# sgl-project/rbg

Hardware: AMD Instinct MI355X
Metric: output tok/s (llama-3-8b P/D-disagg serving, KV migration over xGMI) (higher is better)
Workload: dtype bf16; 1 GPU; model=llama-3-8b, global_batch=128, seq_len=2048, parallelism=pd1 (1 prefill + 1 decode, prefill colocated with decode0)

## Files before the change

rbg_amd/models/llama.py:

```python
from __future__ import annotations

import math
from dataclasses import dataclass
from typing import Optional

import torch
import torch.nn as nn

from .. import ops
from ..engine.config import ModelConfig
from ..engine.kv_cache import PagedKVCache


@dataclass
class ForwardBatch:
    mode: str
    positions: torch.Tensor
    slot_mapping: torch.Tensor
    cu_seqlens: Optional[torch.Tensor] = None
    cu_seqlens_k: Optional[torch.Tensor] = None
    kv_gather_slots: Optional[torch.Tensor] = None
    block_tables: Optional[torch.Tensor] = None
    context_lens: Optional[torch.Tensor] = None
    decode_num_splits: int = 0
# ... 105 lines not shown
                                 requires_grad=False)
        self.wo = _linear_weight(cfg.hidden_size, full_q, device, dtype, gen,
                                 shard_dim=1, tp_size=tp.size,
                                 tp_rank=tp.rank)
        self.q_out, self.kv_out = q_out, kv_out
        self.q_norm = self.k_norm = None
        if cfg.qk_norm:
            self.q_norm = nn.Parameter(torch.ones(cfg.head_dim, device=device,
                                                  dtype=dtype),
                                       requires_grad=False)
            self.k_norm = nn.Parameter(torch.ones(cfg.head_dim, device=device,
                                                  dtype=dtype),
                                       requires_grad=False)

    def forward(self, x: torch.Tensor, batch: ForwardBatch,
                kv: PagedKVCache, cos_sin: torch.Tensor,
                add_norm=None) -> torch.Tensor:
        T = x.shape[0]
        qkv = ops.linear(x, self.wqkv)
        q = qkv[:, :self.q_out]
        k = qkv[:, self.q_out:self.q_out + self.kv_out]
        v = qkv[:, self.q_out + self.kv_out:]
        if self.q_norm is not None:
            q = ops.rmsnorm(q.contiguous().view(-1, self.head_dim),
                            self.q_norm,
                            self.cfg.rms_eps).view(T, self.q_out)
            k = ops.rmsnorm(k.contiguous().view(-1, self.head_dim),
                            self.k_norm,
                            self.cfg.rms_eps).view(T, self.kv_out)
            v = v.clone(memory_format=torch.contiguous_format)
        key_cache = kv.key_cache(self.layer_idx)
        value_cache = kv.value_cache(self.layer_idx)
        fp8 = kv.fp8
        if fp8:
            ops.rope_store_kv(q, k, v, key_cache, value_cache, cos_sin,
                              batch.positions, batch.slot_mapping,
                              kv.k_scale_log2, kv.v_scale_log2)
        else:
            ops.rope_store_kv(q, k, v, key_cache, value_cache, cos_sin,
                              batch.positions, batch.slot_mapping)
        q3 = q.view(T, self.heads, self.head_dim)
        if batch.mode == "prefill":
            if fp8:
                if batch.kv_gather_slots is None:
                    raise RuntimeError("an fp8 KV pool prefills through the "
                                       "gather path: kv_gather_slots unset")
                k_full = ops.kv_gather_dequant(
                    key_cache, batch.kv_gather_slots, kv.k_scale_log2)
                v_full = ops.kv_gather_dequant(
                    value_cache, batch.kv_gather_slots, kv.v_scale_log2)
                o = ops.prefill_attention(q3, k_full, v_full,
                                          batch.cu_seqlens, self.scale,
                                          batch.cu_seqlens_k)
            elif batch.kv_gather_slots is not None:
                ps = key_cache.shape[2]
                slots = batch.kv_gather_slots.long()
                pages, offs = slots // ps, slots % ps
                k_full = key_cache[pages, :, offs]
                v_full = value_cache[pages, :, offs]
                o = ops.prefill_attention(q3, k_full, v_full,
                                          batch.cu_seqlens, self.scale,
                                          batch.cu_seqlens_k)
            else:
                o = ops.prefill_attention(
                    q3, k.view(T, self.kv_heads, self.head_dim),
                    v.view(T, self.kv_heads, self.head_dim),
                    batch.cu_seqlens, self.scale)
        elif fp8:
            o = ops.decode_attention(q3, key_cache, value_cache,
                                     batch.block_tables, batch.context_lens,
                                     self.scale,
                                     num_splits=batch.decode_num_splits,
                                     k_scale_log2=kv.k_scale_log2,
                                     v_scale_log2=kv.v_scale_log2)
        else:
            o = ops.decode_attention(q3, key_cache, value_cache,
                                     batch.block_tables, batch.context_lens,
                                     self.scale,
                                     num_splits=batch.decode_num_splits)
        o = o.view(T, self.q_out).contiguous()
        if add_norm is not None:
            return ops.linear_add_rmsnorm(o, self.wo, *add_norm)
        return self.tp.all_reduce(ops.linear(o, self.wo))


class LlamaMLP(nn.Module):
    def __init__(self, cfg: ModelConfig, tp: TPContext, device, dtype, gen):
        super().__init__()
        self.tp = tp
        assert cfg.intermediate_size % tp.size == 0
        inter = cfg.intermediate_size // tp.size
        wg = _linear_weight(cfg.intermediate_size, cfg.hidden_size, device,
                            dtype, gen, shard_dim=0, tp_size=tp.size,
                            tp_rank=tp.rank)
        wu = _linear_weight(cfg.intermediate_size, cfg.hidden_size, device,
                            dtype, gen, shard_dim=0, tp_size=tp.size,
                            tp_rank=tp.rank)
        self.w_gate_up = nn.Parameter(torch.cat([wg, wu], dim=0),
                                      requires_grad=False)
        self.w_down = _linear_weight(cfg.hidden_size, cfg.intermediate_size,
                                     device, dtype, gen, shard_dim=1,
                                     tp_size=tp.size, tp_rank=tp.rank)
        self.inter = inter

    def forward(self, x: torch.Tensor, add_norm=None) -> torch.Tensor:
        gu = ops.linear(x, self.w_gate_up)
        h = ops.silu_mul(gu)
        if add_norm is not None:
            return ops.linear_add_rmsnorm(h, self.w_down, *add_norm)
        return self.tp.all_reduce(ops.linear(h, self.w_down))


# ... 135 lines not shown
```

rbg_amd/ops/__init__.py:

```python
from __future__ import annotations

import os

import torch

from . import reference

_hip = None
_hip_err: Exception | None = None
try:
    from . import _hip_ops as _hip
except Exception as e:
    _hip_err = e

HAVE_HIP = _hip is not None


def _check_stale() -> None:
    import hashlib
    here = os.path.dirname(os.path.abspath(__file__))
    stamp = os.path.join(here, "_hip_ops.srchash")
    if not os.path.exists(stamp):
        return
    h = hashlib.sha256()
# ... 117 lines not shown


def kv_gather_dequant(cache, slots, scale_log2: int = 0) -> torch.Tensor:
    if cache.dtype != FP8:
        raise ValueError("kv_gather_dequant needs a float8_e4m3fn cache, "
                         "got %s" % cache.dtype)
    check_kv_scale_log2(scale_log2, "scale_log2")
    if _on_gpu(cache):
        return _require_hip().kv_gather_dequant(cache, slots, scale_log2)
    return reference.kv_gather_dequant(cache, slots, scale_log2)


def pick_decode_splits(num_seqs: int, num_kv_heads: int,
                       max_context: int, variant: int = -1) -> int:
    if variant < 0:
        variant = DECODE_VARIANT
    if variant >= 4:
        per_wg = 2 if variant in (4, 5) else 1
        base = num_kv_heads * ((num_seqs + per_wg - 1) // per_wg)
        by_ctx = max(1, max_context // 32)
    else:
        base = num_seqs * num_kv_heads
        by_ctx = max(1, max_context // 256)
    if base >= 1024:
        return 1
    want = max(1, 1024 // max(base, 1))
    return int(min(want, by_ctx, 16))


DECODE_VARIANT = int(os.environ.get("RBG_DECODE_VARIANT", "4"))
PREFILL_SWZ = int(os.environ.get("RBG_PREFILL_SWZ", "6"))


def decode_attention(q, key_cache, value_cache, block_tables, context_lens,
                     scale: float, num_splits: int = 0,
                     variant: int = -1, k_scale_log2: int = 0,
                     v_scale_log2: int = 0) -> torch.Tensor:
    if _is_fp8_pair(key_cache, value_cache):
        if variant not in (-1, 4):
            raise ValueError("an fp8 KV cache has no decode variant %d: only "
                             "variant 4 reads e4m3" % variant)
        check_kv_scale_log2(k_scale_log2, "kv_k_scale_log2")
        check_kv_scale_log2(v_scale_log2, "kv_v_scale_log2")
        if key_cache.shape[2] != 16 or key_cache.shape[3] != 128:
            raise ValueError("fp8 decode needs page size 16 and head_dim 128, "
                             "got %d and %d" % (key_cache.shape[2],
                                                key_cache.shape[3]))
        if _on_gpu(q):
            if num_splits <= 0:
                max_ctx = (int(context_lens.max().item())
                           if context_lens.numel() else 1)
                num_splits = pick_decode_splits(q.shape[0],
                                                key_cache.shape[1], max_ctx, 4)
            return _require_hip().decode_attention_fp8(
                q, key_cache, value_cache, block_tables, context_lens, scale,
                num_splits, k_scale_log2, v_scale_log2)
        return reference.decode_attention(
            q, key_cache, value_cache, block_tables, context_lens, scale,
            k_scale_log2, v_scale_log2)
    if _on_gpu(q):
        if num_splits <= 0:
            max_ctx = int(context_lens.max().item()) if context_lens.numel() else 1
            num_splits = pick_decode_splits(q.shape[0], key_cache.shape[1],
                                            max_ctx)
        if variant < 0:
            variant = DECODE_VARIANT
        return _require_hip().decode_attention(
            q, key_cache, value_cache, block_tables, context_lens, scale,
            num_splits, variant)
    return reference.decode_attention(q, key_cache, value_cache, block_tables,
                                      context_lens, scale)


def prefill_attention(q, k, v, cu_seqlens, scale: float,
                      cu_seqlens_k=None) -> torch.Tensor:
    if _on_gpu(q):
        qtile = 128 if (PREFILL_SWZ & 12) else 64
        block_info, seq_lens = reference.prefill_block_info(
            cu_seqlens.cpu(), qtile=qtile,
            cu_seqlens_k=None if cu_seqlens_k is None else cu_seqlens_k.cpu())
        return _require_hip().prefill_attention(
            q, k, v, block_info.to(q.device), seq_lens.to(q.device), scale,
            PREFILL_SWZ)
    return reference.prefill_attention(q, k, v, cu_seqlens, scale,
                                       cu_seqlens_k)


build_cos_sin_table = reference.build_cos_sin_table


def sample(logits, temperature, top_k, top_p, min_p, seed, pos):
    if _on_gpu(logits):
        toks, kept = _require_hip().sample(logits, temperature, top_k, top_p,
                                           min_p, seed, pos)
        return toks, kept
    return reference.sample(logits, temperature, top_k, top_p, min_p, seed,
                            pos)
```

rbg_amd/ops/hip/attn_decode.hip:

```cpp
#include "attn_mfma.h"

namespace {

struct SplitRange { int key_begin, key_end, pg_begin, pg_end; };

DEV_INLINE SplitRange split_range(int ctx, int split, int num_splits) {
  const int chunk = 16;
  const int nchunks = (ctx + chunk - 1) / chunk;
  const int per_split = (nchunks + num_splits - 1) / num_splits;
  SplitRange r;
  r.key_begin = split * per_split * chunk;
  r.key_end = min(ctx, (split + 1) * per_split * chunk);
  r.pg_begin = r.key_begin >> 4;
  r.pg_end = (r.key_end + 15) >> 4;
  return r;
}

template <int QPG, int VARIANT>
__global__ __launch_bounds__(256,
    (VARIANT == 3) ? 4 : ((VARIANT >= 1 && QPG <= 4) ? 5 : 2))
void decode_attn_kernel(
    float* __restrict__ partial_o,
    float* __restrict__ partial_ml,
    __hip_bfloat16* __restrict__ out,
    const __hip_bfloat16* __restrict__ q,
    const __hip_bfloat16* __restrict__ key_cache,
    const __hip_bfloat16* __restrict__ val_cache,
    const int* __restrict__ block_tables,
    const int* __restrict__ context_lens,
    const float scale, const int num_kv_heads, const int page_size,
    const int max_pages, const int num_splits, const int q_stride) {
  const int kvh = blockIdx.x;
  const int seq = blockIdx.y;
  const int split = blockIdx.z;
  const int num_q_heads = num_kv_heads * QPG;
// ... 303 lines not shown
    }
  }
}

#define DM_REGS(R) uint4 R##0, R##1, R##2, R##3, R##4, R##5, R##6, R##7
#define DM_ISSUE(cache, R, pg)                                              \
  do {                                                                      \
    const int p_ = btab[min((pg) + myloc, pg_last)];                        \
    const __hip_bfloat16* src_ = (cache) + schunk +                         \
        (((size_t)p_ * num_kv_heads + kvh) * 16 + (srow & 15)) * HEAD_DIM;  \
    R##0 = *reinterpret_cast<const uint4*>(src_);                           \
    R##1 = *reinterpret_cast<const uint4*>(src_ + 8);                       \
    R##2 = *reinterpret_cast<const uint4*>(src_ + 16);                      \
    R##3 = *reinterpret_cast<const uint4*>(src_ + 24);                      \
    R##4 = *reinterpret_cast<const uint4*>(src_ + 32);                      \
    R##5 = *reinterpret_cast<const uint4*>(src_ + 40);                      \
    R##6 = *reinterpret_cast<const uint4*>(src_ + 48);                      \
    R##7 = *reinterpret_cast<const uint4*>(src_ + 56);                      \
  } while (0)
#define DM_K_AT(c) (&k_lds[srow * DM_KP + schunk + (c)])
#define DM_V_AT(c) (&v_img[v_img_off(srow, schunk + (c))])
#define DM_WRITE(R, AT)                                                     \
  do {                                                                      \
    *reinterpret_cast<uint4*>(AT(0)) = R##0;                                \
    *reinterpret_cast<uint4*>(AT(8)) = R##1;                                \
    *reinterpret_cast<uint4*>(AT(16)) = R##2;                               \
    *reinterpret_cast<uint4*>(AT(24)) = R##3;                               \
    *reinterpret_cast<uint4*>(AT(32)) = R##4;                               \
    *reinterpret_cast<uint4*>(AT(40)) = R##5;                               \
    *reinterpret_cast<uint4*>(AT(48)) = R##6;                               \
    *reinterpret_cast<uint4*>(AT(56)) = R##7;                               \
  } while (0)

template <int QPG, int DIET>
__global__ __launch_bounds__(128, DIET ? 4 : 3) void decode_attn_mfma_kernel(
    float* __restrict__ partial_o,
    float* __restrict__ partial_ml,
    __hip_bfloat16* __restrict__ out,
    const __hip_bfloat16* __restrict__ q,
    const __hip_bfloat16* __restrict__ key_cache,
    const __hip_bfloat16* __restrict__ val_cache,
    const int* __restrict__ block_tables,
    const int* __restrict__ context_lens,
    const float scale, const int num_kv_heads, const int max_pages,
    const int num_splits, const int num_seqs, const int q_stride) {
  const int kvh = blockIdx.x;
  const int wave = threadIdx.x >> 6;
  const int seq = blockIdx.y * 2 + wave;
  const int split = blockIdx.z;
  const int lane = threadIdx.x & 63;
  const int gl = lane & 15;
  const int gslice = lane >> 4;

  __shared__ __hip_bfloat16 kv_all[2][32 * DM_KP];
  __shared__ __hip_bfloat16 p_lds_all[2][16 * DM_PP];
  __hip_bfloat16* k_lds = kv_all[wave];
  __hip_bfloat16* v_img = kv_all[wave];
  __hip_bfloat16* p_lds = p_lds_all[wave];
  if (seq >= num_seqs) return;
  const SplitRange sr = split_range(context_lens[seq], split, num_splits);

  const __hip_bfloat16* q_seq = q + (size_t)seq * q_stride;
  bf8 qa[4];
  if constexpr (!DIET) load_q_frags<QPG>(qa, q_seq, kvh, gl, gslice);

  const int* btab = block_tables + (size_t)seq * max_pages;
  const int srow = lane >> 1, schunk = (lane & 1) * 64, myloc = srow >> 4;
  const int pg_last = max(sr.pg_end - 1, 0);
  DM_REGS(ka);

  float m[4], l[4];
  f32x4 acc_o[8];
#pragma unroll
  for (int r = 0; r < 4; ++r) { m[r] = NEG_INF; l[r] = 0.f; }
#pragma unroll
  for (int dt = 0; dt < 8; ++dt) acc_o[dt] = {0.f, 0.f, 0.f, 0.f};

  DM_ISSUE(key_cache, ka, sr.pg_begin);

  for (int pg = sr.pg_begin; pg < sr.pg_end; pg += 2) {
    if constexpr (DIET) load_q_frags<QPG>(qa, q_seq, kvh, gl, gslice);
    DM_WRITE(ka, DM_K_AT);
    DM_REGS(va);
    if constexpr (!DIET) DM_ISSUE(val_cache, va, pg);
    asm volatile("s_waitcnt lgkmcnt(0)" ::: "memory");

    f32x4 sA, sB;
    score_pair(sA, sB, qa, k_lds, gl, gslice);
    if constexpr (DIET) DM_ISSUE(val_cache, va, pg);

    pair_softmax(sA, sB, scale, pg, sr, m, l, acc_o, p_lds, gl, gslice);
    DM_WRITE(va, DM_V_AT);
    DM_ISSUE(key_cache, ka, pg + 2);
    asm volatile("s_waitcnt lgkmcnt(0)" ::: "memory");

    const bf8 pa = load_p_frag(p_lds, gl, gslice);
    const unsigned vaddr = v_img_lane_addr(v_img, gl, gslice);
    if constexpr (!DIET) {
      PV_STEP16(acc_o, pa, vaddr);
    } else {
      PV_STEP8(acc_o, pa, vaddr, 0);
      PV_STEP8(acc_o, pa, vaddr, 1);
    }
  }

  store_pair_output<QPG>(partial_o, partial_ml, out, acc_o, m, l, seq,
                         num_seqs, split, num_splits, kvh, num_kv_heads, gl,
                         gslice);
}

template <int QPG>
__global__ __launch_bounds__(128, 4) void decode_attn_pc_kernel(
    float* __restrict__ partial_o,
    float* __restrict__ partial_ml,
    __hip_bfloat16* __restrict__ out,
    const __hip_bfloat16* __restrict__ q,
    const __hip_bfloat16* __restrict__ key_cache,
    const __hip_bfloat16* __restrict__ val_cache,
    const int* __restrict__ block_tables,
    const int* __restrict__ context_lens,
    const float scale, const int num_kv_heads, const int max_pages,
    const int num_splits, const int num_seqs, const int q_stride) {
  const int kvh = blockIdx.x;
  const int seq = blockIdx.y;
  const int split = blockIdx.z;
  const int wave = threadIdx.x >> 6;
  const int lane = threadIdx.x & 63;
  const int gl = lane & 15;
  const int gslice = lane >> 4;

  __shared__ __hip_bfloat16 k_lds[32 * DM_KP];
  __shared__ __hip_bfloat16 v_img[32 * 128];
  __shared__ __hip_bfloat16 p_lds[16 * DM_PP];
  __shared__ int flags[4];
  if (threadIdx.x == 0) {
    flags[0] = -1; flags[1] = -1; flags[2] = -1; flags[3] = -1;
  }
  __syncthreads();
  volatile int* f_prod_k = &flags[0];
  volatile int* f_prod_v = &flags[1];
  volatile int* f_cons_s = &flags[2];
// ... 180 lines not shown
#pragma unroll
    for (int r = 0; r < 4; ++r) acc_o[dt][r] *= v_scale;

  store_pair_output<QPG>(partial_o, partial_ml, out, acc_o, m, l, seq,
                         num_seqs, split, num_splits, kvh, num_kv_heads, gl,
                         gslice);
}

#undef DQ_REGS
#undef DQ_ISSUE
#undef DQ_WRITE1
#undef DQ_WRITE
#undef DM_REGS
#undef DM_ISSUE
#undef DM_K_AT
#undef DM_V_AT
#undef DM_WRITE

__global__ void decode_combine_kernel(
    __hip_bfloat16* __restrict__ out,
    const float* __restrict__ partial_o,
    const float* __restrict__ partial_ml,
    const int num_splits, const int num_q_heads) {
  const int seq = blockIdx.x, qh = blockIdx.y, d = threadIdx.x;
  const int seqs = gridDim.x;
  float m_star = NEG_INF;
  for (int s = 0; s < num_splits; ++s)
    m_star = fmaxf(m_star,
                   partial_ml[(((size_t)s * seqs + seq) * num_q_heads + qh) * 2]);
  float o = 0.f, lsum = 0.f;
  for (int s = 0; s < num_splits; ++s) {
    const float* ml =
        partial_ml + (((size_t)s * seqs + seq) * num_q_heads + qh) * 2;
    const float f = __expf(ml[0] - m_star);
    o += partial_o[(((size_t)s * seqs + seq) * num_q_heads + qh) * HEAD_DIM +
                   d] * f;
    lsum += ml[1] * f;
  }
  out[((size_t)seq * num_q_heads + qh) * HEAD_DIM + d] =
      f2bf(lsum > 0.f ? o / lsum : 0.f);
}

typedef void (*DecodeKernel)(float*, float*, __hip_bfloat16*,
                             const __hip_bfloat16*, const __hip_bfloat16*,
                             const __hip_bfloat16*, const int*, const int*,
                             float, int, int, int, int, int);

template <int QPG>
DecodeKernel decode_kernel(int variant) {
  switch (variant) {
    case 0: return decode_attn_kernel<QPG, 0>;
    case 1: return decode_attn_kernel<QPG, 1>;
    case 2: return decode_attn_kernel<QPG, 2>;
    case 3: return decode_attn_kernel<QPG, 3>;
    case 4: return decode_attn_mfma_kernel<QPG, 0>;
    case 5: return decode_attn_mfma_kernel<QPG, 1>;
    case 6: return decode_attn_pc_kernel<QPG>;
    default: return nullptr;
  }
}

}

extern "C" {

void launch_decode_attention(void* out, void* partial_o, void* partial_ml,
                             const void* q, const void* key_cache,
                             const void* val_cache, const void* block_tables,
                             const void* context_lens, float scale,
                             int num_seqs, int num_q_heads, int num_kv_heads,
                             int page_size, int max_pages, int num_splits,
                             int variant, int q_stride, hipStream_t stream) {
  const int qpg = num_q_heads / num_kv_heads;
  const bool mfma = variant >= 4 && variant <= 6 && page_size == 16;
  const int v = (mfma || (variant >= 0 && variant <= 3)) ? variant : 1;
  const DecodeKernel kernel = qpg == 1   ? decode_kernel<1>(v)
                              : qpg == 2 ? decode_kernel<2>(v)
                              : qpg == 4 ? decode_kernel<4>(v)
                              : qpg == 8 ? decode_kernel<8>(v)
                                         : nullptr;
  if (kernel == nullptr) return;
  const int seq_blocks = (v == 4 || v == 5) ? (num_seqs + 1) / 2 : num_seqs;
  const dim3 grid(num_kv_heads, seq_blocks, num_splits);
  const dim3 block(mfma ? 128 : 256);
  hipLaunchKernelGGL(kernel, grid, block, 0, stream, (float*)partial_o,
                     (float*)partial_ml, (__hip_bfloat16*)out,
                     (const __hip_bfloat16*)q,
                     (const __hip_bfloat16*)key_cache,
                     (const __hip_bfloat16*)val_cache,
                     (const int*)block_tables, (const int*)context_lens,
                     scale, num_kv_heads, mfma ? max_pages : page_size,
                     mfma ? num_splits : max_pages,
                     mfma ? num_seqs : num_splits, q_stride);
  if (num_splits > 1) {
    dim3 cgrid(num_seqs, num_q_heads), cblock(HEAD_DIM);
    hipLaunchKernelGGL(decode_combine_kernel, cgrid, cblock, 0, stream,
                       (__hip_bfloat16*)out, (const float*)partial_o,
// ... 41 lines not shown
```

rbg_amd/ops/hip/bindings.cpp:

```cpp
#include <torch/extension.h>
#include <ATen/hip/HIPContext.h>

#include <hip/hip_runtime.h>

#include <algorithm>
#include <cmath>
#include <cstring>
#include <vector>

extern "C" {
void launch_rmsnorm(void*, void*, const void*, float, int, int, hipStream_t);
void launch_fused_add_rmsnorm(void*, void*, const void*, float, int, int,
                              hipStream_t);
void launch_silu_mul(void*, const void*, int, int, hipStream_t);
void launch_rope_store_kv(void*, void*, const void*, void*, void*,
                          const void*, const void*, const void*, int, int,
                          int, int, int, int, int, hipStream_t);
void launch_decode_attention(void*, void*, void*, const void*, const void*,
                             const void*, const void*, const void*, float,
                             int, int, int, int, int, int, int, int,
                             hipStream_t);
void launch_prefill_attention(void*, const void*, const void*, const void*,
                              const void*, const void*, float, int, int, int,
                              int, int, int, hipStream_t);
void launch_mfma_probe(void*, const void*, const void*, int, int, hipStream_t);
void launch_mfma_probe32(void*, const void*, const void*, int, int, int,
                         hipStream_t);
void launch_skinny_gemm(void*, void*, const void*, const void*, int, int,
                        int, int, hipStream_t);
void launch_skinny_gemm_wide(void*, void*, const void*, const void*, int, int,
                             int, int, hipStream_t);
void launch_reduce_splits(void*, const void*, int, long, hipStream_t);
void launch_fold_add_rmsnorm(void*, const void*, void*, const void*, float,
                             int, int, int, hipStream_t);
void launch_kv_peer_copy(void*, const void*, const void*, const void*, int,
                         int, int, long, long, long, long, hipStream_t);
void launch_xgmi_allreduce(void*, const void*, void**, void**, int, int,
                           long, hipStream_t);
void launch_sample(void*, void*, const void*, const void*, const void*,
                   const void*, const void*, const void*, const void*, int,
                   int, hipStream_t);
void launch_rope_store_kv_fp8(void*, void*, const void*, void*, void*,
                              const void*, const void*, const void*, int, int,
                              int, int, int, int, float, float, hipStream_t);
void launch_kv_gather_dequant(void*, const void*, const void*, long, int, int,
                              int, float, hipStream_t);
void launch_decode_attention_fp8(void*, void*, void*, const void*, const void*,
                                 const void*, const void*, const void*, float,
                                 float, int, int, int, int, int, int,
                                 hipStream_t);
long xgmi_allreduce_signal_bytes();
long xgmi_allreduce_error_offset();
long xgmi_allreduce_counter_offset();
}
// ... 113 lines not shown
  TORCH_CHECK(cos_sin.is_cuda() && cos_sin.is_contiguous() &&
              cos_sin.dim() == 2, "cos_sin must be a contiguous 2-D GPU tensor");
  const int tokens = q.size(0);
  const int head_dim = key_cache.size(3);
  const int num_kv_heads = key_cache.size(1);
  const int page_size = key_cache.size(2);
  TORCH_CHECK(cos_sin.size(1) == head_dim,
              "cos_sin row width must equal the cache head_dim");
  TORCH_CHECK(k.size(0) == tokens && v.size(0) == tokens &&
              positions.numel() == tokens && slot_mapping.numel() == tokens,
              "q/k/v/positions/slot_mapping token counts differ");
  const int64_t q_width = q.numel() / std::max(tokens, 1);
  const int64_t k_width = k.numel() / std::max(tokens, 1);
  const int64_t v_width = v.numel() / std::max(tokens, 1);
  TORCH_CHECK(k_width == (int64_t)num_kv_heads * head_dim && v_width == k_width,
              "k/v rows must be cache KVH * head_dim wide");
  TORCH_CHECK(q_width % head_dim == 0,
              "q row width must be a multiple of the cache head_dim");
  if (tokens == 0) return;
  const int num_q_heads = (int)(q_width / head_dim);
  launch_rope_store_kv(q.data_ptr(), k.data_ptr(), v.data_ptr(),
                       key_cache.data_ptr(), value_cache.data_ptr(),
                       cos_sin.data_ptr(), positions.data_ptr(),
                       slot_mapping.data_ptr(), tokens, num_q_heads,
                       num_kv_heads, head_dim, page_size,
                       (int)q.stride(0), (int)k.stride(0),
                       current_stream());
}

torch::Tensor decode_attention(torch::Tensor q, torch::Tensor key_cache,
                               torch::Tensor value_cache,
                               torch::Tensor block_tables,
                               torch::Tensor context_lens, double scale,
                               int64_t num_splits, int64_t variant) {
  TORCH_CHECK(q.is_cuda() && q.scalar_type() == torch::kBFloat16 &&
              q.dim() == 3 && q.stride(2) == 1 &&
              q.stride(1) == q.size(2), "q must be [T, QH, D] row-sliced");
  const int num_seqs = q.size(0);
  const int num_q_heads = q.size(1);
  const int head_dim = q.size(2);
  TORCH_CHECK(head_dim == 128, "head_dim must be 128");
  check_kv_caches(key_cache, value_cache);
  TORCH_CHECK(key_cache.size(3) == 128, "cache head_dim must be 128");
  const int num_kv_heads = key_cache.size(1);
  const int page_size = key_cache.size(2);
  TORCH_CHECK(num_q_heads % num_kv_heads == 0,
              "q heads must be a multiple of the cache KV heads");
  const int qpg = num_q_heads / num_kv_heads;
  TORCH_CHECK(qpg == 1 || qpg == 2 || qpg == 4 || qpg == 8,
              "GQA group must be 1/2/4/8");
  check_i32_gpu(block_tables, "block_tables");
  check_i32_gpu(context_lens, "context_lens");
  TORCH_CHECK(block_tables.dim() == 2 && block_tables.size(0) == num_seqs,
              "block_tables must be [num_seqs, max_pages]");
  TORCH_CHECK(context_lens.dim() == 1 && context_lens.size(0) == num_seqs,
              "context_lens must be [num_seqs]");
  TORCH_CHECK(num_splits >= 1, "num_splits must be >= 1");
  const int max_pages = block_tables.size(1);
  auto out = torch::empty({num_seqs, num_q_heads, head_dim}, q.options());
  if (num_seqs == 0) return out;
  torch::Tensor partial_o, partial_ml;
  void *po = nullptr, *pml = nullptr;
  if (num_splits > 1) {
    auto opts = q.options().dtype(torch::kFloat32);
    partial_o = torch::empty({num_splits, num_seqs, num_q_heads, head_dim}, opts);
    partial_ml = torch::empty({num_splits, num_seqs, num_q_heads, 2}, opts);
    po = partial_o.data_ptr();
    pml = partial_ml.data_ptr();
  }
  launch_decode_attention(out.data_ptr(), po, pml, q.data_ptr(),
                          key_cache.data_ptr(), value_cache.data_ptr(),
                          block_tables.data_ptr(), context_lens.data_ptr(),
                          (float)scale, num_seqs, num_q_heads, num_kv_heads,
                          page_size, max_pages, (int)num_splits, (int)variant,
                          (int)q.stride(0), current_stream());
  return out;
}


float check_scale_log2(int64_t e, const char* name) {
  TORCH_CHECK(e >= -16 && e <= 16, name, " must be in [-16, 16], got ", e);
  return std::ldexp(1.0f, (int)e);
}

void check_fp8_cache(const torch::Tensor& t, const char* name) {
  TORCH_CHECK(t.is_cuda(), name, " must be on GPU");
  TORCH_CHECK(t.scalar_type() == torch::kFloat8_e4m3fn, name,
              " must be float8_e4m3fn");
  TORCH_CHECK(t.is_contiguous(), name, " must be contiguous");
  TORCH_CHECK(t.dim() == 4, name,
              " must be [pages, KVH, page_size, head_dim]");
  const int64_t page_size = t.size(2);
  TORCH_CHECK(page_size > 0 && (page_size & (page_size - 1)) == 0,
              "page_size must be a power of two");
  TORCH_CHECK(t.size(1) > 0, "cache needs at least one KV head");
  TORCH_CHECK(t.size(3) == 128, "fp8 cache head_dim must be 128");
  TORCH_CHECK(t.numel() / 128 <= INT32_MAX, "cache has too many slots");
}

void check_fp8_caches(const torch::Tensor& key_cache,
                      const torch::Tensor& value_cache) {
// ... 443 lines not shown
  auto t = torch::empty({n}, torch::TensorOptions().dtype(torch::kInt32));
  (void)hipMemcpy(t.data_ptr(), reinterpret_cast<void*>(sig_ptr), n * 4,
                  hipMemcpyDeviceToHost);
  return t;
}

torch::Tensor xgmi_allreduce(torch::Tensor inp,
                             std::vector<int64_t> sig_ptrs,
                             std::vector<int64_t> data_ptrs, int64_t rank) {
  check_bf16_contig(inp, "inp");
  const int world = (int)sig_ptrs.size();
  TORCH_CHECK(world >= 1 && world <= 8 &&
                  data_ptrs.size() == (size_t)world && rank >= 0 &&
                  rank < world,
              "bad world/rank");
  TORCH_CHECK(inp.numel() % 8 == 0, "numel must be a multiple of 8");
  auto out = torch::empty_like(inp);
  void* sp[8];
  void* dp[8];
  for (int i = 0; i < world; ++i) {
    sp[i] = reinterpret_cast<void*>(sig_ptrs[i]);
    dp[i] = reinterpret_cast<void*>(data_ptrs[i]);
  }
  launch_xgmi_allreduce(out.data_ptr(), inp.data_ptr(), sp, dp, world,
                        (int)rank, (long)inp.numel(), current_stream());
  return out;
}

PYBIND11_MODULE(TORCH_EXTENSION_NAME, m) {
  m.def("rmsnorm", &rmsnorm, "RMSNorm (bf16)");
  m.def("fused_add_rmsnorm", &fused_add_rmsnorm, "x,residual += ; rmsnorm");
  m.def("silu_mul", &silu_mul, "silu(gate)*up");
  m.def("rope_store_kv", &rope_store_kv, "RoPE + paged KV write");
  m.def("decode_attention", &decode_attention, "paged flash-decode");
  m.def("rope_store_kv_fp8", &rope_store_kv_fp8,
        "RoPE + quantising (e4m3) paged KV write");
  m.def("kv_gather_dequant", &kv_gather_dequant,
        "gather e4m3 cache rows by slot -> bf16 [Tkv, KVH, D]");
  m.def("decode_attention_fp8", &decode_attention_fp8,
        "paged flash-decode over an e4m3 cache (page-pair MFMA)");
  m.def("prefill_attention", &prefill_attention, "varlen causal flash prefill");
  m.def("mfma_probe", &mfma_probe, "MFMA layout probe");
  m.def("mfma_probe32", &mfma_probe32, "32x32x16 MFMA layout probe");
  m.def("skinny_gemm", &skinny_gemm, "decode-shape GEMM (M<=128)",
        py::arg("a"), py::arg("w"), py::arg("force_splits") = 0,
        py::arg("panel") = 0);
  m.def("skinny_gemm_add_rmsnorm", &skinny_gemm_add_rmsnorm,
        "skinny_gemm + fused_add_rmsnorm with the split-K fold inside the "
        "norm kernel; returns h, updates residual in place",
        py::arg("a"), py::arg("w"), py::arg("residual"),
        py::arg("norm_weight"), py::arg("eps"), py::arg("force_splits") = 0,
        py::arg("panel") = 0);
  m.def("sample", &sample,
        "seeded top-k/min-p/top-p Gumbel-max sampler -> (tokens, num_kept)");
  m.def("ipc_alloc_bf16", &ipc_alloc_bf16,
        "hipMalloc-backed bf16 tensor (IPC-exportable base allocation)",
        py::call_guard<py::gil_scoped_release>());
  m.def("ipc_alloc", &ipc_alloc,
        "hipMalloc-backed tensor of any dtype (IPC-exportable allocation)",
        py::call_guard<py::gil_scoped_release>());
  m.def("kv_ipc_export", &kv_ipc_export, "hipIpcGetMemHandle of a KV pool");
  m.def("kv_ipc_open", &kv_ipc_open,
        "map a peer KV pool (lazy xGMI peer access)",
        py::call_guard<py::gil_scoped_release>());
  m.def("kv_ipc_close", &kv_ipc_close, "unmap a peer KV pool",
        py::call_guard<py::gil_scoped_release>());
  m.def("kv_peer_copy", &kv_peer_copy,
// ... 12 lines not shown
```

rbg_amd/ops/hip/rope_kv.hip:

```cpp
#include "common.h"

namespace {

__global__ void rope_store_kv_kernel(
    __hip_bfloat16* __restrict__ q,
    __hip_bfloat16* __restrict__ k,
    const __hip_bfloat16* __restrict__ v,
    __hip_bfloat16* __restrict__ key_cache,
    __hip_bfloat16* __restrict__ val_cache,
    const float* __restrict__ cos_sin,
    const int* __restrict__ positions,
    const int* __restrict__ slot_mapping,
    const int num_q_heads, const int num_kv_heads, const int head_dim,
    const int page_size,
    const int q_stride, const int kv_stride) {
  const int token = blockIdx.x;
  const int tid = threadIdx.x;
  const int pos = positions[token];
  const int slot = slot_mapping[token];
  const int half = head_dim / 2;
  const float* cs = cos_sin + (size_t)pos * head_dim;

  __hip_bfloat16* q_tok = q + (size_t)token * q_stride;
  const int q_pairs = num_q_heads * half;
  for (int i = tid; i < q_pairs; i += blockDim.x) {
    const int h = i / half, d = i % half;
    __hip_bfloat16* base = q_tok + h * head_dim;
    const float x1 = bf2f(base[d]), x2 = bf2f(base[d + half]);
    const float c = cs[d], s = cs[half + d];
    base[d] = f2bf(x1 * c - x2 * s);
    base[d + half] = f2bf(x2 * c + x1 * s);
  }

  __hip_bfloat16* k_tok = k + (size_t)token * kv_stride;
  const __hip_bfloat16* v_tok = v + (size_t)token * kv_stride;
  const int page = slot >= 0 ? slot / page_size : 0;
  const int poff = slot >= 0 ? slot % page_size : 0;
  const int kv_pairs = num_kv_heads * half;
  for (int i = tid; i < kv_pairs; i += blockDim.x) {
    const int h = i / half, d = i % half;
    __hip_bfloat16* base = k_tok + h * head_dim;
    const float x1 = bf2f(base[d]), x2 = bf2f(base[d + half]);
    const float c = cs[d], s = cs[half + d];
    const __hip_bfloat16 r1 = f2bf(x1 * c - x2 * s);
    const __hip_bfloat16 r2 = f2bf(x2 * c + x1 * s);
    base[d] = r1;
    base[d + half] = r2;
    if (slot >= 0) {
      __hip_bfloat16* kdst = key_cache +
          (((size_t)page * num_kv_heads + h) * page_size + poff) * head_dim;
      kdst[d] = r1;
      kdst[d + half] = r2;
    }
  }
  if (slot >= 0) {
    const int nvec = num_kv_heads * head_dim / 8;
    for (int i = tid; i < nvec; i += blockDim.x) {
      const int h = (i * 8) / head_dim;
      const int d = (i * 8) % head_dim;
      __hip_bfloat16* vdst = val_cache +
          (((size_t)page * num_kv_heads + h) * page_size + poff) * head_dim;
      *reinterpret_cast<uint4*>(vdst + d) =
          *reinterpret_cast<const uint4*>(v_tok + h * head_dim + d);
    }
  }
}

}

extern "C" {

void launch_rope_store_kv(void* q, void* k, const void* v, void* key_cache,
                          void* val_cache, const void* cos_sin,
                          const void* positions, const void* slot_mapping,
                          int tokens, int num_q_heads, int num_kv_heads,
                          int head_dim, int page_size, int q_stride,
                          int kv_stride, hipStream_t stream) {
  dim3 grid(tokens), block(256);
// ... 11 lines not shown
```

Baseline: 10940 tok/s.

## Fuse RoPE and KV-cache write into decode attention, pair splits in-block

For bf16 decode with variant 4, RoPE on q/k and the paged K/V store now run inside the decode attention kernel instead of a separate rope_store_kv launch. The split that owns the last key writes the new token to the cache, with a workgroup fence, before it loads that page. A new paired mode handles two splits as two waves of one block and combines them through LDS. This drops the separate combine kernel and the partial buffers when num_splits is 2. The aim is fewer launches and less global traffic per decode layer, at the cost of more kernel complexity and a cross-wave ordering risk on the freshly written cache slot.

```diff
diff --git a/rbg_amd/models/llama.py b/rbg_amd/models/llama.py
--- a/rbg_amd/models/llama.py
+++ b/rbg_amd/models/llama.py
@@ -161,7 +161,11 @@
         key_cache = kv.key_cache(self.layer_idx)
         value_cache = kv.value_cache(self.layer_idx)
         fp8 = kv.fp8
-        if fp8:
+        rope = None
+        if (batch.mode != "prefill" and not fp8 and
+                ops.decode_fuses_rope(q, key_cache)):
+            rope = (k, v, cos_sin, batch.positions, batch.slot_mapping)
+        elif fp8:
             ops.rope_store_kv(q, k, v, key_cache, value_cache, cos_sin,
                               batch.positions, batch.slot_mapping,
                               kv.k_scale_log2, kv.v_scale_log2)
@@ -206,7 +210,8 @@
             o = ops.decode_attention(q3, key_cache, value_cache,
                                      batch.block_tables, batch.context_lens,
                                      self.scale,
-                                     num_splits=batch.decode_num_splits)
+                                     num_splits=batch.decode_num_splits,
+                                     rope=rope)
         o = o.view(T, self.q_out).contiguous()
         if add_norm is not None:
             return ops.linear_add_rmsnorm(o, self.wo, *add_norm)
diff --git a/rbg_amd/ops/__init__.py b/rbg_amd/ops/__init__.py
--- a/rbg_amd/ops/__init__.py
+++ b/rbg_amd/ops/__init__.py
@@ -173,11 +173,27 @@
 PREFILL_SWZ = int(os.environ.get("RBG_PREFILL_SWZ", "6"))
 
 
+DECODE_FUSE_ROPE = int(os.environ.get("RBG_DECODE_FUSE_ROPE", "1"))
+DECODE_PAIR = int(os.environ.get("RBG_DECODE_PAIR", "1"))
+
+
+def decode_fuses_rope(q, key_cache) -> bool:
+    return bool(DECODE_FUSE_ROPE and _on_gpu(q) and
+                key_cache.dtype == torch.bfloat16 and DECODE_VARIANT == 4 and
+                key_cache.shape[2] == 16 and key_cache.shape[3] == 128)
+
+
 def decode_attention(q, key_cache, value_cache, block_tables, context_lens,
                      scale: float, num_splits: int = 0,
                      variant: int = -1, k_scale_log2: int = 0,
-                     v_scale_log2: int = 0) -> torch.Tensor:
+                     v_scale_log2: int = 0, rope=None) -> torch.Tensor:
+    if rope is not None and len(rope) != 5:
+        raise ValueError("rope must be (k, v, cos_sin, positions, "
+                         "slot_mapping)")
     if _is_fp8_pair(key_cache, value_cache):
+        if rope is not None:
+            raise ValueError("rope cannot be fused into decode over an fp8 "
+                             "KV cache")
         if variant not in (-1, 4):
             raise ValueError("an fp8 KV cache has no decode variant %d: only "
                              "variant 4 reads e4m3" % variant)
@@ -206,9 +222,18 @@
                                             max_ctx)
         if variant < 0:
             variant = DECODE_VARIANT
+        if rope is None:
+            return _require_hip().decode_attention(
+                q, key_cache, value_cache, block_tables, context_lens, scale,
+                num_splits, variant, pair=bool(DECODE_PAIR))
         return _require_hip().decode_attention(
             q, key_cache, value_cache, block_tables, context_lens, scale,
-            num_splits, variant)
+            num_splits, variant, *rope, pair=bool(DECODE_PAIR))
+    if rope is not None:
+        k, v, cos_sin, positions, slot_mapping = rope
+        q, k = q.clone(), k.clone()
+        reference.rope_store_kv(q.view(q.shape[0], -1), k, v, key_cache,
+                                value_cache, cos_sin, positions, slot_mapping)
     return reference.decode_attention(q, key_cache, value_cache, block_tables,
                                       context_lens, scale)
 
diff --git a/rbg_amd/ops/hip/attn_decode.hip b/rbg_amd/ops/hip/attn_decode.hip
--- a/rbg_amd/ops/hip/attn_decode.hip
+++ b/rbg_amd/ops/hip/attn_decode.hip
@@ -1,6 +1,27 @@
 #include "attn_mfma.h"
+#include "rope_rotate.h"
 
 namespace {
+
+DEV_INLINE void combine_fold(float& o, float& lsum, float part_o, float m,
+                             float l, float m_star) {
+  const float f = __expf(m - m_star);
+  o = __builtin_fmaf(part_o, f, o);
+  lsum = __builtin_fmaf(l, f, lsum);
+}
+
+DEV_INLINE __hip_bfloat16 combine_finish(float o, float lsum) {
+  return f2bf(lsum > 0.f ? o / lsum : 0.f);
+}
+
+struct DecodeRopeArgs {
+  const __hip_bfloat16* k;
+  const __hip_bfloat16* v;
+  const float* cos_sin;
+  const int* positions;
+  const int* slot_mapping;
+  int kv_stride;
+};
 
 struct SplitRange { int key_begin, key_end, pg_begin, pg_end; };
 
@@ -370,6 +391,179 @@
     *reinterpret_cast<uint4*>(AT(56)) = R##7;                               \
   } while (0)
 
+template <int QPG, int DIET, int FUSE, int PAIR, typename CacheT>
+DEV_INLINE void decode_mfma_body(
+    float* partial_o, float* partial_ml, __hip_bfloat16* out,
+    const __hip_bfloat16* q, CacheT* key_cache, CacheT* val_cache,
+    const int* block_tables, const int* context_lens, const float scale,
+    const int num_kv_heads, const int max_pages, const int num_splits_arg,
+    const int num_seqs, const int q_stride, const DecodeRopeArgs& rope) {
+  const int kvh = blockIdx.x;
+  const int wave = threadIdx.x >> 6;
+  const int seq = PAIR ? blockIdx.y : blockIdx.y * 2 + wave;
+  const int split = PAIR ? wave : blockIdx.z;
+  const int num_splits = PAIR ? 2 : num_splits_arg;
+  const int lane = threadIdx.x & 63;
+  const int gl = lane & 15;
+  const int gslice = lane >> 4;
+
+  __shared__ __hip_bfloat16 kv_all[2][32 * DM_KP];
+  __shared__ __hip_bfloat16 p_lds_all[2][16 * DM_PP];
+  __hip_bfloat16* k_lds = kv_all[wave];
+  __hip_bfloat16* v_img = kv_all[wave];
+  __hip_bfloat16* p_lds = p_lds_all[wave];
+  if constexpr (!PAIR) {
+    if (seq >= num_seqs) return;
+  }
+  const SplitRange sr = split_range(context_lens[seq], split, num_splits);
+
+  const __hip_bfloat16* q_seq = q + (size_t)seq * q_stride;
+  bf8 qa[4];
+  if constexpr (!DIET) load_q_frags<QPG>(qa, q_seq, kvh, gl, gslice);
+
+  const int* btab = block_tables + (size_t)seq * max_pages;
+  const int srow = lane >> 1, schunk = (lane & 1) * 64, myloc = srow >> 4;
+  const int pg_last = max(sr.pg_end - 1, 0);
+  DM_REGS(ka);
+
+  float m[4], l[4];
+  f32x4 acc_o[8];
+#pragma unroll
+  for (int r = 0; r < 4; ++r) { m[r] = NEG_INF; l[r] = 0.f; }
+#pragma unroll
+  for (int dt = 0; dt < 8; ++dt) acc_o[dt] = {0.f, 0.f, 0.f, 0.f};
+
+  if constexpr (FUSE) {
+    const int ctx = context_lens[seq];
+    const int slot = rope.slot_mapping[seq];
+    const float* cs = rope.cos_sin + (size_t)rope.positions[seq] * HEAD_DIM;
+    const bool writer = slot >= 0 &&
+        (ctx == 0 ? split == 0
+                  : (sr.key_begin < sr.key_end && sr.key_end == ctx));
+    const bool write_first = writer && sr.pg_end - sr.pg_begin <= 2;
+
+    float4 cq[2][2], sq[2][2];
+#pragma unroll
+    for (int ks = 0; ks < 2; ++ks) {
+      const float* c = cs + ks * 32 + gslice * 8;
+      cq[ks][0] = *reinterpret_cast<const float4*>(c);
+      cq[ks][1] = *reinterpret_cast<const float4*>(c + 4);
+      sq[ks][0] = *reinterpret_cast<const float4*>(c + 64);
+      sq[ks][1] = *reinterpret_cast<const float4*>(c + 68);
+    }
+    const size_t kv_off = (size_t)seq * rope.kv_stride + kvh * HEAD_DIM;
+    const __hip_bfloat16 k1 = rope.k[kv_off + lane];
+    const __hip_bfloat16 k2 = rope.k[kv_off + 64 + lane];
+    const float kc = cs[lane], ks_ = cs[64 + lane];
+    const unsigned vv =
+        *reinterpret_cast<const unsigned*>(rope.v + kv_off + 2 * lane);
+
+    if (!write_first) DM_ISSUE(key_cache, ka, sr.pg_begin);
+
+#pragma unroll
+    for (int ks = 0; ks < 2; ++ks) {
+      union { bf8 v; __hip_bfloat16 e[8]; } lo, hi;
+      lo.v = qa[ks];
+      hi.v = qa[ks + 2];
+      const float cj[8] = {cq[ks][0].x, cq[ks][0].y, cq[ks][0].z, cq[ks][0].w,
+                           cq[ks][1].x, cq[ks][1].y, cq[ks][1].z, cq[ks][1].w};
+      const float sj[8] = {sq[ks][0].x, sq[ks][0].y, sq[ks][0].z, sq[ks][0].w,
+                           sq[ks][1].x, sq[ks][1].y, sq[ks][1].z, sq[ks][1].w};
+#pragma unroll
+      for (int j = 0; j < 8; ++j)
+        rope_rotate_pair(lo.e[j], hi.e[j], cj[j], sj[j], lo.e[j], hi.e[j]);
+      qa[ks] = lo.v;
+      qa[ks + 2] = hi.v;
+    }
+
+    if (writer) {
+      __hip_bfloat16 r1, r2;
+      rope_rotate_pair(k1, k2, kc, ks_, r1, r2);
+      const size_t dst =
+          (((size_t)(slot >> 4) * num_kv_heads + kvh) * 16 + (slot & 15)) *
+          HEAD_DIM;
+      key_cache[dst + lane] = r1;
+      key_cache[dst + 64 + lane] = r2;
+      *reinterpret_cast<unsigned*>(val_cache + dst + 2 * lane) = vv;
+      __builtin_amdgcn_fence(__ATOMIC_RELEASE, "workgroup");
+    }
+    if (write_first) DM_ISSUE(key_cache, ka, sr.pg_begin);
+  } else {
+    DM_ISSUE(key_cache, ka, sr.pg_begin);
+  }
+
+  for (int pg = sr.pg_begin; pg < sr.pg_end; pg += 2) {
+    if constexpr (DIET) load_q_frags<QPG>(qa, q_seq, kvh, gl, gslice);
+    DM_WRITE(ka, DM_K_AT);
+    DM_REGS(va);
+    if constexpr (!DIET) DM_ISSUE(val_cache, va, pg);
+    asm volatile("s_waitcnt lgkmcnt(0)" ::: "memory");
+
+    f32x4 sA, sB;
+    score_pair(sA, sB, qa, k_lds, gl, gslice);
+    if constexpr (DIET) DM_ISSUE(val_cache, va, pg);
+
+    pair_softmax(sA, sB, scale, pg, sr, m, l, acc_o, p_lds, gl, gslice);
+    DM_WRITE(va, DM_V_AT);
+    DM_ISSUE(key_cache, ka, pg + 2);
+    asm volatile("s_waitcnt lgkmcnt(0)" ::: "memory");
+
+    const bf8 pa = load_p_frag(p_lds, gl, gslice);
+    const unsigned vaddr = v_img_lane_addr(v_img, gl, gslice);
+    if constexpr (!DIET) {
+      PV_STEP16(acc_o, pa, vaddr);
+    } else {
+      PV_STEP8(acc_o, pa, vaddr, 0);
+      PV_STEP8(acc_o, pa, vaddr, 1);
+    }
+  }
+
+  if constexpr (PAIR) {
+    float* xch = reinterpret_cast<float*>(kv_all[1]);
+    float* xch_ml = xch + 32 * 64;
+    static_assert((32 * 64 + 32) * sizeof(float) <=
+                  32 * DM_KP * sizeof(__hip_bfloat16), "panel too small");
+    if (wave == 1) {
+#pragma unroll
+      for (int r = 0; r < 4; ++r) {
+        if (4 * gslice + r >= QPG) continue;
+#pragma unroll
+        for (int dt = 0; dt < 8; ++dt)
+          xch[(dt * 4 + r) * 64 + lane] = acc_o[dt][r];
+        if (gl == 0) {
+          xch_ml[(4 * gslice + r) * 2] = m[r];
+          xch_ml[(4 * gslice + r) * 2 + 1] = l[r];
+        }
+      }
+    }
+    __syncthreads();
+    if (wave == 0) {
+      const int num_q_heads = num_kv_heads * QPG;
+#pragma unroll
+      for (int r = 0; r < 4; ++r) {
+        const int row = 4 * gslice + r;
+        if (row >= QPG) continue;
+        const float m1 = xch_ml[row * 2], l1 = xch_ml[row * 2 + 1];
+        const float m_star = fmaxf(fmaxf(NEG_INF, m[r]), m1);
+        __hip_bfloat16* orow =
+            out + ((size_t)seq * num_q_heads + kvh * QPG + row) * HEAD_DIM;
+#pragma unroll
+        for (int dt = 0; dt < 8; ++dt) {
+          float o = 0.f, lsum = 0.f;
+          combine_fold(o, lsum, acc_o[dt][r], m[r], l[r], m_star);
+          combine_fold(o, lsum, xch[(dt * 4 + r) * 64 + lane], m1, l1,
+                       m_star);
+          orow[dt * 16 + gl] = combine_finish(o, lsum);
+        }
+      }
+    }
+  } else {
+    store_pair_output<QPG>(partial_o, partial_ml, out, acc_o, m, l, seq,
+                           num_seqs, split, num_splits, kvh, num_kv_heads, gl,
+                           gslice);
+  }
+}
+
 template <int QPG, int DIET>
 __global__ __launch_bounds__(128, DIET ? 4 : 3) void decode_attn_mfma_kernel(
     float* __restrict__ partial_o,
@@ -382,69 +576,29 @@
     const int* __restrict__ context_lens,
     const float scale, const int num_kv_heads, const int max_pages,
     const int num_splits, const int num_seqs, const int q_stride) {
-  const int kvh = blockIdx.x;
-  const int wave = threadIdx.x >> 6;
-  const int seq = blockIdx.y * 2 + wave;
-  const int split = blockIdx.z;
-  const int lane = threadIdx.x & 63;
-  const int gl = lane & 15;
-  const int gslice = lane >> 4;
-
-  __shared__ __hip_bfloat16 kv_all[2][32 * DM_KP];
-  __shared__ __hip_bfloat16 p_lds_all[2][16 * DM_PP];
-  __hip_bfloat16* k_lds = kv_all[wave];
-  __hip_bfloat16* v_img = kv_all[wave];
-  __hip_bfloat16* p_lds = p_lds_all[wave];
-  if (seq >= num_seqs) return;
-  const SplitRange sr = split_range(context_lens[seq], split, num_splits);
-
-  const __hip_bfloat16* q_seq = q + (size_t)seq * q_stride;
-  bf8 qa[4];
-  if constexpr (!DIET) load_q_frags<QPG>(qa, q_seq, kvh, gl, gslice);
-
-  const int* btab = block_tables + (size_t)seq * max_pages;
-  const int srow = lane >> 1, schunk = (lane & 1) * 64, myloc = srow >> 4;
-  const int pg_last = max(sr.pg_end - 1, 0);
-  DM_REGS(ka);
-
-  float m[4], l[4];
-  f32x4 acc_o[8];
-#pragma unroll
-  for (int r = 0; r < 4; ++r) { m[r] = NEG_INF; l[r] = 0.f; }
-#pragma unroll
-  for (int dt = 0; dt < 8; ++dt) acc_o[dt] = {0.f, 0.f, 0.f, 0.f};
-
-  DM_ISSUE(key_cache, ka, sr.pg_begin);
-
-  for (int pg = sr.pg_begin; pg < sr.pg_end; pg += 2) {
-    if constexpr (DIET) load_q_frags<QPG>(qa, q_seq, kvh, gl, gslice);
-    DM_WRITE(ka, DM_K_AT);
-    DM_REGS(va);
-    if constexpr (!DIET) DM_ISSUE(val_cache, va, pg);
-    asm volatile("s_waitcnt lgkmcnt(0)" ::: "memory");
-
-    f32x4 sA, sB;
-    score_pair(sA, sB, qa, k_lds, gl, gslice);
-    if constexpr (DIET) DM_ISSUE(val_cache, va, pg);
-
-    pair_softmax(sA, sB, scale, pg, sr, m, l, acc_o, p_lds, gl, gslice);
-    DM_WRITE(va, DM_V_AT);
-    DM_ISSUE(key_cache, ka, pg + 2);
-    asm volatile("s_waitcnt lgkmcnt(0)" ::: "memory");
-
-    const bf8 pa = load_p_frag(p_lds, gl, gslice);
-    const unsigned vaddr = v_img_lane_addr(v_img, gl, gslice);
-    if constexpr (!DIET) {
-      PV_STEP16(acc_o, pa, vaddr);
-    } else {
-      PV_STEP8(acc_o, pa, vaddr, 0);
-      PV_STEP8(acc_o, pa, vaddr, 1);
-    }
-  }
-
-  store_pair_output<QPG>(partial_o, partial_ml, out, acc_o, m, l, seq,
-                         num_seqs, split, num_splits, kvh, num_kv_heads, gl,
-                         gslice);
+  decode_mfma_body<QPG, DIET, 0, 0>(
+      partial_o, partial_ml, out, q, key_cache, val_cache, block_tables,
+      context_lens, scale, num_kv_heads, max_pages, num_splits, num_seqs,
+      q_stride, DecodeRopeArgs{});
+}
+
+template <int QPG, int FUSE, int PAIR>
+__global__ __launch_bounds__(128, 3) void decode_attn_mfma_fused_kernel(
+    float* __restrict__ partial_o,
+    float* __restrict__ partial_ml,
+    __hip_bfloat16* __restrict__ out,
+    const __hip_bfloat16* __restrict__ q,
+    __hip_bfloat16* key_cache,
+    __hip_bfloat16* val_cache,
+    const int* __restrict__ block_tables,
+    const int* __restrict__ context_lens,
+    const float scale, const int num_kv_heads, const int max_pages,
+    const int num_splits, const int num_seqs, const int q_stride,
+    const DecodeRopeArgs rope) {
+  decode_mfma_body<QPG, 0, FUSE, PAIR>(
+      partial_o, partial_ml, out, q, key_cache, val_cache, block_tables,
+      context_lens, scale, num_kv_heads, max_pages, num_splits, num_seqs,
+      q_stride, rope);
 }
 
 template <int QPG>
@@ -691,13 +845,13 @@
   for (int s = 0; s < num_splits; ++s) {
     const float* ml =
         partial_ml + (((size_t)s * seqs + seq) * num_q_heads + qh) * 2;
-    const float f = __expf(ml[0] - m_star);
-    o += partial_o[(((size_t)s * seqs + seq) * num_q_heads + qh) * HEAD_DIM +
-                   d] * f;
-    lsum += ml[1] * f;
+    combine_fold(o, lsum,
+                 partial_o[(((size_t)s * seqs + seq) * num_q_heads + qh) *
+                               HEAD_DIM + d],
+                 ml[0], ml[1], m_star);
   }
   out[((size_t)seq * num_q_heads + qh) * HEAD_DIM + d] =
-      f2bf(lsum > 0.f ? o / lsum : 0.f);
+      combine_finish(o, lsum);
 }
 
 typedef void (*DecodeKernel)(float*, float*, __hip_bfloat16*,
@@ -719,9 +873,63 @@
   }
 }
 
+typedef void (*DecodeFusedKernel)(float*, float*, __hip_bfloat16*,
+                                  const __hip_bfloat16*, __hip_bfloat16*,
+                                  __hip_bfloat16*, const int*, const int*,
+                                  float, int, int, int, int, int,
+                                  DecodeRopeArgs);
+
+template <int QPG>
+DecodeFusedKernel decode_fused_kernel(bool fuse, bool pair) {
+  if (fuse && pair) return decode_attn_mfma_fused_kernel<QPG, 1, 1>;
+  if (fuse) return decode_attn_mfma_fused_kernel<QPG, 1, 0>;
+  if (pair) return decode_attn_mfma_fused_kernel<QPG, 0, 1>;
+  return nullptr;
+}
+
 }
 
 extern "C" {
+
+void launch_decode_attention_fused(
+    void* out, void* partial_o, void* partial_ml, const void* q,
+    void* key_cache, void* val_cache, const void* block_tables,
+    const void* context_lens, float scale, int num_seqs, int num_q_heads,
+    int num_kv_heads, int max_pages, int num_splits, int q_stride,
+    const void* k, const void* v, const void* cos_sin, const void* positions,
+    const void* slot_mapping, int kv_stride, int pair, hipStream_t stream) {
+  const int qpg = num_q_heads / num_kv_heads;
+  const bool fuse = k != nullptr;
+  const bool pr = pair != 0 && num_splits == 2;
+  const DecodeFusedKernel kernel =
+      qpg == 1   ? decode_fused_kernel<1>(fuse, pr)
+      : qpg == 2 ? decode_fused_kernel<2>(fuse, pr)
+      : qpg == 4 ? decode_fused_kernel<4>(fuse, pr)
+      : qpg == 8 ? decode_fused_kernel<8>(fuse, pr)
+                 : nullptr;
+  if (kernel == nullptr) return;
+  DecodeRopeArgs rope;
+  rope.k = (const __hip_bfloat16*)k;
+  rope.v = (const __hip_bfloat16*)v;
+  rope.cos_sin = (const float*)cos_sin;
+  rope.positions = (const int*)positions;
+  rope.slot_mapping = (const int*)slot_mapping;
+  rope.kv_stride = kv_stride;
+  const dim3 grid = pr ? dim3(num_kv_heads, num_seqs, 1)
+                       : dim3(num_kv_heads, (num_seqs + 1) / 2, num_splits);
+  hipLaunchKernelGGL(kernel, grid, dim3(128), 0, stream, (float*)partial_o,
+                     (float*)partial_ml, (__hip_bfloat16*)out,
+                     (const __hip_bfloat16*)q, (__hip_bfloat16*)key_cache,
+                     (__hip_bfloat16*)val_cache, (const int*)block_tables,
+                     (const int*)context_lens, scale, num_kv_heads, max_pages,
+                     num_splits, num_seqs, q_stride, rope);
+  if (!pr && num_splits > 1) {
+    dim3 cgrid(num_seqs, num_q_heads), cblock(HEAD_DIM);
+    hipLaunchKernelGGL(decode_combine_kernel, cgrid, cblock, 0, stream,
+                       (__hip_bfloat16*)out, (const float*)partial_o,
+                       (const float*)partial_ml, num_splits, num_q_heads);
+  }
+}
 
 void launch_decode_attention(void* out, void* partial_o, void* partial_ml,
                              const void* q, const void* key_cache,
diff --git a/rbg_amd/ops/hip/bindings.cpp b/rbg_amd/ops/hip/bindings.cpp
--- a/rbg_amd/ops/hip/bindings.cpp
+++ b/rbg_amd/ops/hip/bindings.cpp
@@ -20,6 +20,11 @@
                              const void*, const void*, const void*, float,
                              int, int, int, int, int, int, int, int,
                              hipStream_t);
+void launch_decode_attention_fused(void*, void*, void*, const void*, void*,
+                                   void*, const void*, const void*, float,
+                                   int, int, int, int, int, int, const void*,
+                                   const void*, const void*, const void*,
+                                   const void*, int, int, hipStream_t);
 void launch_prefill_attention(void*, const void*, const void*, const void*,
                               const void*, const void*, float, int, int, int,
                               int, int, int, hipStream_t);
@@ -199,7 +204,13 @@
                                torch::Tensor value_cache,
                                torch::Tensor block_tables,
                                torch::Tensor context_lens, double scale,
-                               int64_t num_splits, int64_t variant) {
+                               int64_t num_splits, int64_t variant,
+                               c10::optional<torch::Tensor> rope_k,
+                               c10::optional<torch::Tensor> rope_v,
+                               c10::optional<torch::Tensor> cos_sin,
+                               c10::optional<torch::Tensor> positions,
+                               c10::optional<torch::Tensor> slot_mapping,
+                               bool pair) {
   TORCH_CHECK(q.is_cuda() && q.scalar_type() == torch::kBFloat16 &&
               q.dim() == 3 && q.stride(2) == 1 &&
               q.stride(1) == q.size(2), "q must be [T, QH, D] row-sliced");
@@ -224,16 +235,67 @@
               "context_lens must be [num_seqs]");
   TORCH_CHECK(num_splits >= 1, "num_splits must be >= 1");
   const int max_pages = block_tables.size(1);
+  const bool fuse = rope_k.has_value();
+  TORCH_CHECK(fuse == rope_v.has_value() && fuse == cos_sin.has_value() &&
+              fuse == positions.has_value() &&
+              fuse == slot_mapping.has_value(),
+              "rope needs all of k, v, cos_sin, positions, slot_mapping");
+  if (fuse) {
+    TORCH_CHECK(variant == 4, "rope is fused into decode variant 4 only, got ",
+                variant);
+    TORCH_CHECK(page_size == 16, "fused rope needs page size 16, got ",
+                page_size);
+    const torch::Tensor &k = *rope_k, &v = *rope_v;
+    check_bf16_rowslice(k, "rope k");
+    check_bf16_rowslice(v, "rope v");
+    TORCH_CHECK(k.size(0) == num_seqs && v.size(0) == num_seqs,
+                "rope k/v must have one row per sequence");
+    TORCH_CHECK(k.numel() == (int64_t)num_seqs * num_kv_heads * head_dim &&
+                v.numel() == k.numel(),
+                "rope k/v rows must be cache KVH * head_dim wide");
+    TORCH_CHECK(k.stride(0) == v.stride(0), "rope k/v stride mismatch");
+    TORCH_CHECK(k.stride(0) % 8 == 0 && q.stride(0) % 8 == 0 &&
+                k.storage_offset() % 8 == 0 && v.storage_offset() % 8 == 0,
+                "rope q/k/v rows must be 16-byte aligned");
+    TORCH_CHECK(k.device() == q.device() && v.device() == q.device(),
+                "rope k/v device mismatch");
+    TORCH_CHECK(cos_sin->is_cuda() && cos_sin->is_contiguous() &&
+                cos_sin->dim() == 2 &&
+                cos_sin->scalar_type() == torch::kFloat32 &&
+                cos_sin->size(1) == head_dim,
+                "cos_sin must be a contiguous fp32 [max_pos, head_dim] GPU "
+                "tensor");
+    check_i32_gpu(*positions, "positions");
+    check_i32_gpu(*slot_mapping, "slot_mapping");
+    TORCH_CHECK(positions->numel() == num_seqs &&
+                slot_mapping->numel() == num_seqs,
+                "positions/slot_mapping must have one entry per sequence");
+  }
   auto out = torch::empty({num_seqs, num_q_heads, head_dim}, q.options());
   if (num_seqs == 0) return out;
+  const bool pr = pair && num_splits == 2 && variant == 4 && page_size == 16;
   torch::Tensor partial_o, partial_ml;
   void *po = nullptr, *pml = nullptr;
-  if (num_splits > 1) {
+  if (num_splits > 1 && !pr) {
     auto opts = q.options().dtype(torch::kFloat32);
     partial_o = torch::empty({num_splits, num_seqs, num_q_heads, head_dim}, opts);
     partial_ml = torch::empty({num_splits, num_seqs, num_q_heads, 2}, opts);
     po = partial_o.data_ptr();
     pml = partial_ml.data_ptr();
+  }
+  if (fuse || pr) {
+    launch_decode_attention_fused(
+        out.data_ptr(), po, pml, q.data_ptr(), key_cache.data_ptr(),
+        value_cache.data_ptr(), block_tables.data_ptr(),
+        context_lens.data_ptr(), (float)scale, num_seqs, num_q_heads,
+        num_kv_heads, max_pages, (int)num_splits, (int)q.stride(0),
+        fuse ? rope_k->data_ptr() : nullptr,
+        fuse ? rope_v->data_ptr() : nullptr,
+        fuse ? cos_sin->data_ptr() : nullptr,
+        fuse ? positions->data_ptr() : nullptr,
+        fuse ? slot_mapping->data_ptr() : nullptr,
+        fuse ? (int)rope_k->stride(0) : 0, pr ? 1 : 0, current_stream());
+    return out;
   }
   launch_decode_attention(out.data_ptr(), po, pml, q.data_ptr(),
                           key_cache.data_ptr(), value_cache.data_ptr(),
@@ -743,7 +805,13 @@
   m.def("fused_add_rmsnorm", &fused_add_rmsnorm, "x,residual += ; rmsnorm");
   m.def("silu_mul", &silu_mul, "silu(gate)*up");
   m.def("rope_store_kv", &rope_store_kv, "RoPE + paged KV write");
-  m.def("decode_attention", &decode_attention, "paged flash-decode");
+  m.def("decode_attention", &decode_attention, "paged flash-decode",
+        py::arg("q"), py::arg("key_cache"), py::arg("value_cache"),
+        py::arg("block_tables"), py::arg("context_lens"), py::arg("scale"),
+        py::arg("num_splits"), py::arg("variant"),
+        py::arg("rope_k") = py::none(), py::arg("rope_v") = py::none(),
+        py::arg("cos_sin") = py::none(), py::arg("positions") = py::none(),
+        py::arg("slot_mapping") = py::none(), py::arg("pair") = false);
   m.def("rope_store_kv_fp8", &rope_store_kv_fp8,
         "RoPE + quantising (e4m3) paged KV write");
   m.def("kv_gather_dequant", &kv_gather_dequant,
diff --git a/rbg_amd/ops/hip/rope_kv.hip b/rbg_amd/ops/hip/rope_kv.hip
--- a/rbg_amd/ops/hip/rope_kv.hip
+++ b/rbg_amd/ops/hip/rope_kv.hip
@@ -1,4 +1,5 @@
 #include "common.h"
+#include "rope_rotate.h"
 
 namespace {
 
@@ -26,10 +27,10 @@
   for (int i = tid; i < q_pairs; i += blockDim.x) {
     const int h = i / half, d = i % half;
     __hip_bfloat16* base = q_tok + h * head_dim;
-    const float x1 = bf2f(base[d]), x2 = bf2f(base[d + half]);
-    const float c = cs[d], s = cs[half + d];
-    base[d] = f2bf(x1 * c - x2 * s);
-    base[d + half] = f2bf(x2 * c + x1 * s);
+    __hip_bfloat16 r1, r2;
+    rope_rotate_pair(base[d], base[d + half], cs[d], cs[half + d], r1, r2);
+    base[d] = r1;
+    base[d + half] = r2;
   }
 
   __hip_bfloat16* k_tok = k + (size_t)token * kv_stride;
@@ -40,10 +41,8 @@
   for (int i = tid; i < kv_pairs; i += blockDim.x) {
     const int h = i / half, d = i % half;
     __hip_bfloat16* base = k_tok + h * head_dim;
-    const float x1 = bf2f(base[d]), x2 = bf2f(base[d + half]);
-    const float c = cs[d], s = cs[half + d];
-    const __hip_bfloat16 r1 = f2bf(x1 * c - x2 * s);
-    const __hip_bfloat16 r2 = f2bf(x2 * c + x1 * s);
+    __hip_bfloat16 r1, r2;
+    rope_rotate_pair(base[d], base[d + half], cs[d], cs[half + d], r1, r2);
     base[d] = r1;
     base[d + half] = r2;
     if (slot >= 0) {
diff --git a/rbg_amd/ops/hip/rope_rotate.h b/rbg_amd/ops/hip/rope_rotate.h
--- /dev/null
+++ b/rbg_amd/ops/hip/rope_rotate.h
@@ -0,0 +1,11 @@
+#pragma once
+
+#include "common.h"
+
+DEV_INLINE void rope_rotate_pair(__hip_bfloat16 a, __hip_bfloat16 b, float c,
+                                 float s, __hip_bfloat16& r1,
+                                 __hip_bfloat16& r2) {
+  const float x1 = bf2f(a), x2 = bf2f(b);
+  r1 = f2bf(__builtin_fmaf(x1, c, -(x2 * s)));
+  r2 = f2bf(__builtin_fmaf(x2, c, x1 * s));
+}
```

Result: no change. 10930 tok/s (-0.1%).
